# mpriessner/MultiModalSpectralTransformer

Hardware: NVIDIA B200
Metric: generated SMILES tokens/sec (higher is better)
Workload: dtype bf16

## Files before the change

multimodalspectraltransformer_b200/csrc/engine.cu:

```cuda
#include "engine.cuh"
#include "kernels_simt.cuh"
#include "kernels_tc.cuh"
#include "kernels_decode.cuh"
#include "kernels_ffn.cuh"
#include "kernels_attn5.cuh"
#include "kernels_compact.cuh"
#include "kernels_beam.cuh"
#include "kernels_smiles.cuh"
#include "kernels_retire.cuh"

#include <algorithm>
#include <cstdlib>
#include <cstring>

namespace mmt {
thread_local std::string g_last_error;

static const char* kEmbedKeys[5] = {
    "linear_spec_embedding_1H.point_embedding_layer_1H.fc_H",
    "linear_spec_embedding_13C.point_embedding_layer_13C.fc_C",
    "linear_spec_embedding_HSQC.point_embedding_layer_HSQC.fc_HSQC",
    "linear_spec_embedding_COSY.point_embedding_layer_COSY.fc_COSY",
    "linear_spec_embedding_IR.linear_spec_embedding_IR"};
static const char* kEncNames[6] = {"encoder_1H", "encoder_13C", "encoder_HSQC", "encoder_COSY", "encoder_IR", "encoder_cross"};
// ... 811 lines not shown
        }
    }
    {
        EncGroupRun g;
        memset(&g, 0, sizeof(g));
        g.X = b.Xc; g.rows = Bc * L.S_total; g.S = L.S_total; g.kbias = key_bias; g.kidx = b.kidx_c; g.nk = b.nk_c;
        g.qkv = b.QKV; g.att = b.ATT; g.part = b.PART; g.h = b.H;
        g.x16 = b.Xc16; g.att16 = b.ATT16; g.h16 = b.H16;
        for (int l = 0; l < d.n_enc_layers; ++l) {
            g.w = &e->enc[5][l];
            if (l == d.n_enc_layers - 1) { g.out = d_memory; g.out16 = nullptr; g.stride_b = 1; g.stride_s = B_total; g.off = b0; }
            if (bf16) MMT_TRY(encoder_layer_bf16(e, &g, 1, Bc, d.n_heads_cross, d.d_ff, s));
            else MMT_TRY(encoder_layer_fp32(e, &g, 1, Bc, d.n_heads_cross, d.d_ff, s));
        }
    }
    return 0;
}

struct DecBuffers {
    float *x, *qkv, *att, *part, *qc, *h;
    int64_t part_rows;
    char* kv_pool; int* block_table;
    int64_t pool_pages;
    char* cross_kv;
    size_t kv_esz;
    int *nk, *row_start; int64_t* row_off; float* kbias_c;
    int* ctl;
    uint64_t* rng_state;
    __nv_bfloat16 *x16, *att16, *h16, *mem16;
    int64_t plan_rows;
    const int *orig, *col_start, *col_count;
    int* eos_len;
    int *rt_orig[2], *rt_bt, *rt_src, *rt_col_start, *rt_col_count;
};
constexpr int MAX_SPLITS = 32;

static void plan_decoder(Arena& a, const mmt_model_desc& d, int64_t Nw, int Bmw, int S, int max_len, DecBuffers& b, bool bf16, int fused_rows, int kv_copies = 1,
                         bool retire = false) {
    const int L = d.n_dec_layers;
    const int pps = (max_len + PAGE_TOKENS - 1) / PAGE_TOKENS;
    b.x = a.get<float>(Nw * D);
    b.qkv = a.get<float>(Nw * 3 * D);
    b.att = a.get<float>(Nw * D);
    b.part_rows = std::max<int64_t>(Nw, std::min<int64_t>(Nw, std::max(fused_rows, 2048)) * MAX_SPLITS);
    b.part = a.get<float>(b.part_rows * D);
    b.qc = a.get<float>(Nw * D);
    b.h = a.get<float>(bf16 ? 0 : Nw * d.d_ff);
    b.kv_esz = bf16 ? 2 : 4;
    b.pool_pages = (int64_t)kv_copies * Nw * pps;
    b.kv_pool = a.get<char>((size_t)L * b.pool_pages * 2 * PAGE_TOKENS * D * b.kv_esz);
    b.block_table = a.get<int>(Nw * pps);
    int64_t R = (int64_t)Bmw * S;
    b.cross_kv = a.get<char>((size_t)L * 2 * R * D * b.kv_esz);
    b.nk = a.get<int>(Bmw);
    b.row_start = a.get<int>(Bmw);
    b.row_off = a.get<int64_t>(R);
    b.kbias_c = a.get<float>(R);
    b.ctl = a.get<int>(8 + 256);
    b.rng_state = a.get<uint64_t>(2);
    b.x16 = b.att16 = b.h16 = b.mem16 = nullptr;
    if (bf16) {
        b.x16 = a.get<__nv_bfloat16>(Nw * D);
        b.att16 = a.get<__nv_bfloat16>(Nw * D);
        b.h16 = nullptr;
        b.mem16 = a.get<__nv_bfloat16>(R * D);
    }
    b.plan_rows = 0; b.orig = b.col_start = b.col_count = nullptr; b.eos_len = nullptr;
    b.rt_orig[0] = b.rt_orig[1] = b.rt_bt = b.rt_src = b.rt_col_start = b.rt_col_count = nullptr;
    if (retire) {
        b.rt_orig[0] = a.get<int>(Nw); b.rt_orig[1] = a.get<int>(Nw); b.rt_bt = a.get<int>(Nw * pps); b.rt_src = a.get<int>(Nw);
        b.rt_col_start = a.get<int>(Bmw); b.rt_col_count = a.get<int>(Bmw);
    }
}

__global__ void init_block_table(int* bt, int64_t Nw, int pps) {
    int64_t i = (int64_t)blockIdx.x * blockDim.x + threadIdx.x;
    if (i < Nw * pps) bt[i] = (int)((i % pps) * Nw + i / pps);
}

struct DecodeRun {
    const mmt_decode_args* a;
    int mode;
    const int64_t* trg;
    const int64_t* target = nullptr; float* target_prob = nullptr;
    int T;
    int64_t* tokens; float* probs; float* logits;
    int64_t ldn = -1;
    bool serial_first = false;
    bool per_memory_rng = false;
    int64_t eos = -1;
    int32_t* len = nullptr;
    int64_t* h_rows = nullptr;
};

static int decode_prepare_wave(mmt_engine* e, const mmt_decode_args& a, int b0, int Bmw, DecBuffers& b, bool bf16, cudaStream_t s) {
// ... 12 lines not shown
        pack_rows_bf16<<<(unsigned)((R + 7) / 8), 256, 0, s>>>(a.d_memory + (int64_t)b0 * a.stride_b, b.row_off, 0, R, b.mem16);
        MMT_TRY(check_launch(e, "pack_rows_bf16", s));
        for (int l = 0; l < d.n_dec_layers; ++l) {
            TcGemmParams p = tc_params((int)R, 2 * D, D);
            p.bias = e->dec[l].ca_in_b + D;
            p.out_b16 = reinterpret_cast<__nv_bfloat16*>(b.cross_kv + (size_t)l * 2 * R * D * b.kv_esz);
            p.head_major = 1; p.hm_heads = d.n_heads; p.hm_dh = dh; p.hm_rows = a.S;
            MMT_TRY(launch_tc(e, p, b.mem16, D, e->Wb(e->dec[l].ca_in_w + (int64_t)D * D), TC_EPI_STORE, s, e->Wlo(e->dec[l].ca_in_w + (int64_t)D * D)));
        }
        return 0;
    }
    for (int l = 0; l < d.n_dec_layers; ++l) {
        GemmParams p = gemm_params(2 * D, D, 0, 0);
        p.g[0].A = a.d_memory + (int64_t)b0 * a.stride_b; p.g[0].a_row_off = b.row_off; p.g[0].lda = 0;
        p.g[0].W = e->dec[l].ca_in_w + (int64_t)D * D;
        p.g[0].bias = e->dec[l].ca_in_b + D;
        p.g[0].C = reinterpret_cast<float*>(b.cross_kv + (size_t)l * 2 * R * D * b.kv_esz); p.g[0].M = (int)R;
        p.out_mode = GEMM_OUT_HEADMAJOR; p.hm_heads = d.n_heads; p.hm_dh = dh; p.hm_rows = a.S;
        MMT_TRY(launch_gemm(e, p, 1, (int)R, s));
    }
    return 0;
}

static int decode_self_attention_layer(mmt_engine* e, const LayerW& w, const DecBuffers& b, char* pool, int pps, int64_t Nw, bool bf16,
                                       bool pdl_u, cudaStream_t s) {
    const int H = e->desc.n_heads, dh = D / H;
    const float scale = 1.0f / sqrtf((float)dh);
    const int* step = b.ctl;
    const int M = (int)Nw;
    if (dh != 8) MMT_FAIL("decoder head dim must be 8");
    if (bf16) {
        TcGemmParams p = tc_params(M, 3 * D, D);
        p.bias = w.in_b; p.out_f32 = b.qkv; p.ld_f32 = e->use_kv_epilogue ? D : 3 * D;
        p.kv_append = e->use_kv_epilogue ? (e->kv_tok_major && H % 8 == 0 ? 2 : 1) : 0; p.kv_pool = reinterpret_cast<__nv_bfloat16*>(pool); p.block_table = b.block_table; p.pps = pps; p.step = step; p.kv_heads = H;
        MMT_TRY(launch_tc(e, p, b.x16, D, e->Wb(w.in_w), TC_EPI_STORE, s, e->dec_proj_single ? nullptr : e->Wlo(w.in_w), pdl_u));
    } else {
        GemmParams p = gemm_params(3 * D, D, 3 * D, 0);
        p.g[0].A = b.x; p.g[0].lda = D; p.g[0].W = w.in_w; p.g[0].bias = w.in_b; p.g[0].C = b.qkv; p.g[0].M = M;
        p.splits = 1; p.part_stride = Nw * D;
        MMT_TRY(launch_gemm(e, p, 1, M, s, b.plan_rows));
    }
    prof_pre(e, s);
    const unsigned sa_blocks = (unsigned)((Nw * (H / 4) + 7) / 8);
    if (bf16 && e->use_kv_epilogue && e->kv_tok_major && H % 8 == 0)
        launch_args(decode_self_attention_tm<8>, dim3((unsigned)((Nw * (H / 8) + 7) / 8)), dim3(256), 0, s, pdl_u, (const float*)b.qkv, (const __nv_bfloat16*)reinterpret_cast<__nv_bfloat16*>(pool), (const int*)b.block_table, pps, Nw, H, scale, step, b.att16);
    else if (bf16 && e->use_kv_epilogue) launch_args(decode_self_attention_g8<8, __nv_bfloat16, false>, dim3(sa_blocks), dim3(256), 0, s, pdl_u, (const float*)b.qkv, reinterpret_cast<__nv_bfloat16*>(pool), (const int*)b.block_table, pps, Nw, H, scale, step, (float*)nullptr, b.att16);
    else if (bf16) launch_args(decode_self_attention_g8<8, __nv_bfloat16>, dim3(sa_blocks), dim3(256), 0, s, pdl_u, (const float*)b.qkv, reinterpret_cast<__nv_bfloat16*>(pool), (const int*)b.block_table, pps, Nw, H, scale, step, (float*)nullptr, b.att16);
    else decode_self_attention_g8<8, float><<<sa_blocks, 256, 0, s>>>(b.qkv, reinterpret_cast<float*>(pool), b.block_table, pps, Nw, H, scale, step, b.att, b.att16);
    return check_launch(e, "decode_self_attention", s);
}

static int decode_cross_attention_layer(mmt_engine* e, const mmt_decode_args& a, const DecBuffers& b, const char* ckv, int64_t Nw, int Bmw,
                                        bool bf16, bool pdl_u, cudaStream_t s) {
    const int H = e->desc.n_heads, dh = D / H;
    const float scale = 1.0f / sqrtf((float)dh);
    if (dh != 8) MMT_FAIL("decoder head dim must be 8");
    const unsigned attn_blocks = (unsigned)((Nw * H + 7) / 8);
    prof_pre(e, s);
    if (bf16 && a.n_cand >= 8 && e->use_tc_attention)
        launch_args(decode_cross_attention_tc, dim3(H, Bmw), dim3(256), dx_smem_bytes(a.S), s, pdl_u, (const float*)b.qc, reinterpret_cast<const __nv_bfloat16*>(ckv), (int64_t)a.S, (const int*)b.nk, (const int*)b.row_start, (const float*)b.kbias_c, (int)a.n_cand, H, scale, (float*)nullptr, b.att16, b.col_start, b.col_count);
    else if (bf16) launch_args(decode_cross_attention<8, __nv_bfloat16>, dim3(attn_blocks), dim3(256), 0, s, pdl_u, (const float*)b.qc, reinterpret_cast<const __nv_bfloat16*>(ckv), (int64_t)a.S, (const int*)b.nk, (const int*)b.row_start, (const float*)b.kbias_c, (int)a.n_cand, Nw, H, scale, (float*)nullptr, b.att16, b.orig);
    else decode_cross_attention<8, float><<<attn_blocks, 256, 0, s>>>(b.qc, reinterpret_cast<const float*>(ckv), a.S, b.nk, b.row_start, b.kbias_c, a.n_cand, Nw, H, scale, b.att, b.att16, b.orig);
    return check_launch(e, "decode_cross_attention", s);
}

struct DecOps {
    mmt_engine* e; const DecBuffers& b; int64_t Nw; bool pdl_u; cudaStream_t s;
    int64_t plan() const { return b.plan_rows > 0 ? b.plan_rows : Nw; }
// ... 129 lines not shown
        if (bf16 && e->ffn_splits_override > 0) ffn_splits = e->ffn_splits_override;
        if (!cl_ffn && (int64_t)ffn_splits * Nw > b.part_rows) MMT_FAIL("decode: FFN partial buffer too small for this wave (plan_decoder)");
        if (cl_ffn) ffn_splits = 0;
        for (int l = 0; l < d.n_dec_layers; ++l) {
            const LayerW& w = e->dec[l];
            DecAttnParams q;
            memset(&q, 0, sizeof(q));
            if (l == 0) {
                if (r.trg) { q.tokens = r.trg + n0; q.tok_shift = 0; }
                else { q.tokens = r.tokens + n0; q.tok_shift = 1; }
                q.sos = 3; q.ldn = ldn; q.E_tok = e->W("embed_trg.weight"); q.E_pos = e->W("pe_trg.weight"); q.vocab = d.vocab;
            } else {
                const LayerW& pw = e->dec[l - 1];
                q.x_in = b.x;
                if (!cl_ffn) { q.part = b.part; q.splits = ffn_splits; q.part_stride = Nw * D; q.pbias = pw.l2_b; q.pgamma = pw.n3_w; q.pbeta = pw.n3_b; }
            }
            if (cl_ffn) {
                MMT_TRY(tc_init(e));
                MMT_TRY(make_tmap(&q.tmW1, e->Wb(w.l1_w), d.d_ff, D, D));
                MMT_TRY(make_tmap(&q.tmW2, e->Wb(w.l2_w), D, d.d_ff, d.d_ff));
                q.b1 = w.l1_b; q.b2 = w.l2_b; q.n3_w = w.n3_w; q.n3_b = w.n3_b; q.x_out = b.x;
            }
            q.in_w = w.in_w; q.in_b = w.in_b; q.out_w = w.out_w; q.out_b = w.out_b; q.n1_w = w.n1_w; q.n1_b = w.n1_b;
            q.kv_pool = b.kv_pool + (size_t)l * b.pool_pages * 2 * PAGE_TOKENS * D * b.kv_esz; q.block_table = b.block_table; q.pps = pps;
            q.step = step;
            q.in_w16 = e->Wb(w.in_w); q.out_w16 = e->Wb(w.out_w); q.cq_w16 = e->Wb(w.ca_in_w); q.co_w16 = e->Wb(w.ca_out_w);
            q.cq_w = w.ca_in_w; q.cq_b = w.ca_in_b; q.co_w = w.ca_out_w; q.co_b = w.ca_out_b; q.n2_w = w.n2_w; q.n2_b = w.n2_b;
            q.ckv = b.cross_kv + (size_t)l * 2 * R * D * b.kv_esz; q.rows_total = a.S;
            q.nk = b.nk; q.row_start = b.row_start; q.kbias_c = b.kbias_c; q.n_cand = a.n_cand;
            q.x2 = b.x; q.x2_16 = bf16 ? b.x16 : nullptr; q.M = Nw; q.scale = scale; q.eps = 1e-5f;
            q.dbg = (e->da_dbg && l == 3) ? e->da_dbg : nullptr;
            prof_pre(e, s);
            const bool pdl_l = pdl && !(l == 0 && r.serial_first);
            if (cl_ffn) launch_kernel_cluster(decode_attn<8, __nv_bfloat16, true>, dim3(blocks), dim3(DA_THREADS), DA_SMEM_BYTES_CL, s, pdl_l, DA_CL, q);
            else if (bf16) launch_kernel(decode_attn<8, __nv_bfloat16>, dim3(blocks), dim3(DA_THREADS), DA_SMEM_BYTES, s, pdl_l, q);
            else launch_kernel(decode_attn<8, float>, dim3(blocks), dim3(DA_THREADS), DA_SMEM_BYTES, s, pdl_l, q);
            MMT_TRY(check_launch(e, "decode_attn", s));
            if (cl_ffn) continue;
            if (bf16) {
                FfnParams f = ffn_params(M, d.d_ff);
                f.b1 = w.l1_b; f.splits = ffn_splits; f.out_f32 = b.part; f.part_stride = Nw * D;
                f.dbg = (e->da_dbg && l == 3) ? e->da_dbg + 2048 * 16 : nullptr;
                MMT_TRY(launch_ffn(e, f, b.x16, D, e->Wb(w.l1_w), o.dlo(w.l1_w), e->Wb(w.l2_w), o.dlo(w.l2_w), TC_EPI_STORE, s, pdl));
            } else {
                MMT_TRY(o.gemm(b.x, D, w.l1_w, w.l1_b, b.h, d.d_ff, D, 1, 1));
                MMT_TRY(o.gemm(b.h, d.d_ff, w.l2_w, nullptr, b.part, D, d.d_ff, 0, ffn_splits));
            }
        }
    } else {
        prof_pre(e, s);
        if (r.trg) launch_args(decode_embed, dim3((unsigned)((Nw + 3) / 4)), dim3(128), 0, s, pdl_u, r.trg + n0, 0, 3, Nw, ldn, e->W("embed_trg.weight"), e->W("pe_trg.weight"), (int)d.vocab, step, b.x, b.x16, b.orig);
        else launch_args(decode_embed, dim3((unsigned)((Nw + 3) / 4)), dim3(128), 0, s, pdl_u, (const int64_t*)(r.tokens + n0), 1, 3, Nw, ldn, e->W("embed_trg.weight"), e->W("pe_trg.weight"), (int)d.vocab, step, b.x, b.x16, b.orig);
        MMT_TRY(check_launch(e, "decode_embed", s));

        for (int l = 0; l < d.n_dec_layers; ++l) {
            const LayerW& w = e->dec[l];
            char* pool = b.kv_pool + (size_t)l * b.pool_pages * 2 * PAGE_TOKENS * D * b.kv_esz;
            const char* ckv = b.cross_kv + (size_t)l * 2 * R * D * b.kv_esz;
            MMT_TRY(decode_self_attention_layer(e, w, b, pool, pps, Nw, bf16, pdl_u, s));
            MMT_TRY(decode_self_tail_layer(o, w, bf16));
            MMT_TRY(decode_cross_attention_layer(e, a, b, ckv, Nw, Bmw, bf16, pdl_u, s));
            MMT_TRY(decode_cross_tail_layer(o, w, l, bf16));
        }
    }
    SampleParams sp;
    memset(&sp, 0, sizeof(sp));
    sp.x = b.x; sp.W = e->W("fc_out.weight"); sp.b = e->W("fc_out.bias"); sp.V = d.vocab; sp.N = Nw; sp.ldn = ldn;
    sp.temperature = a.temperature; sp.mode = r.mode;
    int smc = a.rng_sm_count > 0 ? a.rng_sm_count : e->sm_count;
    int mts = a.rng_max_threads_per_sm > 0 ? a.rng_max_threads_per_sm : e->max_threads_per_sm;
    int64_t Nrng = r.per_memory_rng ? a.n_cand : (a.N_total > 0 ? a.N_total : N_total);
    sp.rng.seed = a.philox_seed; sp.rng.offset = a.philox_offset; sp.rng.numel = Nrng * d.vocab;
    sp.rng.threads = torch_rng_threads(sp.rng.numel, smc, mts);
    sp.rng_inc = torch_rng_increment(sp.rng.numel, smc, mts);
    sp.rng_dev = b.rng_state;
    sp.seq_index_base = a.seq_index_base + n0;
    if (r.per_memory_rng) { sp.rng_cand = a.n_cand; sp.rng_col_steps = a.max_len; }
    sp.tokens = r.tokens ? r.tokens + n0 : nullptr; sp.probs = r.probs ? r.probs + n0 : nullptr;
    sp.logits = r.logits ? r.logits + n0 * d.vocab : nullptr;
    sp.target = r.target ? r.target + n0 : nullptr; sp.target_prob = r.target_prob ? r.target_prob + n0 : nullptr;
    sp.ctl.step = b.ctl; sp.ctl.done_ctas = b.ctl + 1; sp.ctl.nonpad = (r.mode == 0) ? b.ctl + 8 : nullptr;
    sp.advance = 1;
// ... 26 lines not shown
    const int64_t N_total = (int64_t)a.Bm * a.n_cand;
    const int64_t max_wave_seqs = e->max_wave_seqs > 0 ? e->max_wave_seqs
                                  : (a.precision == MMT_PREC_BF16 ? (int64_t)e->sm_count * (e->total_mem >= ((size_t)128 << 30) ? 8 : 4) * 128 : 32768);
    int Bm_wave = (int)std::max<int64_t>(1, std::min<int64_t>(a.Bm, max_wave_seqs / a.n_cand));
    const int n_waves = (a.Bm + Bm_wave - 1) / Bm_wave;
    if (a.precision != MMT_PREC_FP32 && a.precision != MMT_PREC_BF16) MMT_FAIL("decode: bad precision");
    const bool bf16 = a.precision == MMT_PREC_BF16;
    constexpr int MAX_LANES = 4;
    int NL = 1;
    {
        const int64_t Nwave = (int64_t)Bm_wave * a.n_cand;
        const bool fused = e->fused_decode_rows > 0 && Nwave <= e->fused_decode_rows;
        if (fused && e->use_graph && !e->profiling) {
            NL = std::min(std::min(e->decode_lanes, MAX_LANES), Bm_wave);
            while (NL > 1 && Nwave / NL < 32) --NL;
        } else if (!fused && bf16 && e->use_graph && !e->profiling && Nwave >= 4096) {
            NL = std::min(std::min(e->decode_lanes_large, MAX_LANES), Bm_wave);
        }
    }
    const int Bm_lane = (Bm_wave + NL - 1) / NL;
    const bool retire = r.eos >= 0;
    const bool small_wave = e->fused_decode_rows > 0 && (int64_t)Bm_wave * a.n_cand <= e->fused_decode_rows;
    const bool staged = e->use_graph && e->use_graph_cache && !e->profiling && n_waves == 1 && r.mode != 2 && !r.trg && (!retire || small_wave);
    Arena ar;
    DecBuffers lb[MAX_LANES];
    int64_t* st_tokens = nullptr; float* st_probs = nullptr;
    int* eos_all = nullptr;
    auto plan_all = [&]() {
        for (int i = 0; i < NL; ++i) plan_decoder(ar, d, (int64_t)Bm_lane * a.n_cand, Bm_lane, a.S, a.max_len, lb[i], bf16, e->fused_decode_rows, 1, retire);
        if (staged) { st_tokens = ar.get<int64_t>((size_t)a.max_len * N_total); st_probs = ar.get<float>((size_t)a.max_len * N_total); }
        if (retire) eos_all = ar.get<int>(N_total);
    };
    ar.plan = true;
    plan_all();
    MMT_TRY(ensure_arena(e, ar.off));
    ar.plan = false; ar.base = e->arena; ar.cap = e->arena_bytes; ar.off = 0;
    plan_all();
    DecodeRun rs = r;
    if (staged) { rs.tokens = st_tokens; rs.probs = r.probs ? st_probs : nullptr; }
    const int pps = (a.max_len + PAGE_TOKENS - 1) / PAGE_TOKENS;
    const bool early = (r.mode == 0) && a.stop_on_all_pad && n_waves == 1;
    int steps_done = r.T;
    std::vector<int64_t> nonpad_total(r.T, 0);
    std::vector<int64_t> live_total(r.T, 0), rows_at(r.T, 0);
    if (retire) {
        fill_i32<<<(unsigned)((N_total + 255) / 256), 256, 0, s>>>(eos_all, N_total, a.max_len);
        MMT_CUDA(cudaGetLastError());
        for (int i = 0; i < 2; ++i) if (!e->poll_ev[i]) MMT_CUDA(cudaEventCreateWithFlags(&e->poll_ev[i], cudaEventDisableTiming));
    }
    for (int wv = 0; wv < n_waves; ++wv) {
        const int wb0 = wv * Bm_wave;
        const int Bmw = std::min(Bm_wave, a.Bm - wb0);
// ... 379 lines not shown
    if (prop.major != 10) MMT_FAIL(std::string("device is sm_") + std::to_string(prop.major * 10 + prop.minor) + "; this library is built for sm_100a (B200) only");
    MMT_CUDA(cudaSetDevice(device));
    mmt_engine* e = new mmt_engine();
    e->desc = *desc; e->device = device; e->sm_count = prop.multiProcessorCount; e->max_threads_per_sm = prop.maxThreadsPerMultiProcessor; e->total_mem = prop.totalGlobalMem;
    e->reg = build_registry(*desc);
    if (getenv("MMT_NO_GRAPH")) e->use_graph = false;
    if (getenv("MMT_NO_PDL")) e->use_pdl = false;
    if (getenv("MMT_NO_GRAPH_CACHE")) e->use_graph_cache = false;
    if (const char* v = getenv("MMT_GRAPH_STEPS")) e->graph_steps = std::max(1, atoi(v));
    if (getenv("MMT_NO_ENC_STREAMS")) e->use_enc_streams = false;
    if (const char* v = getenv("MMT_DECODE_LANES")) e->decode_lanes = std::max(1, atoi(v));
    if (getenv("MMT_DENSE_ENCODER")) e->use_compact = false;
    if (getenv("MMT_NO_TC_ATTENTION")) e->use_tc_attention = false;
    if (getenv("MMT_TC5_ATTENTION")) e->use_tc5_attention = true;
    if (const char* v = getenv("MMT_FFN_SPLITS")) { int k = atoi(v); if (k == 1 || k == 2 || k == 4 || k == 8 || k == 16 || k == 32) e->ffn_splits_override = k; }
    if (getenv("MMT_TC_ATTENTION_FP32")) e->tc_attention_fp32 = true;
    if (const char* v = getenv("MMT_FUSED_DECODE_ROWS")) e->fused_decode_rows = atoi(v);
    if (getenv("MMT_DEC_FFN_TWO_TERM")) e->dec_ffn_single = false;
    if (getenv("MMT_DEC_PROJ_TWO_TERM")) e->dec_proj_single = false;
    if (const char* v = getenv("MMT_PDL_ROWS")) e->pdl_rows = atoi(v);
    if (getenv("MMT_NO_GEMM_CHAIN")) e->use_gemm_chain = false;
    if (getenv("MMT_NO_FFN_WIDE")) e->use_ffn_wide = false;
    if (getenv("MMT_NO_KV_EPILOGUE")) e->use_kv_epilogue = false;
    if (getenv("MMT_KV_HEAD_MAJOR")) e->kv_tok_major = false;
    if (getenv("MMT_CLUSTER_FFN")) e->use_cluster_ffn = true;
    if (getenv("MMT_NO_FFN_PROLOGUE")) e->use_ffn_prologue = false;
    if (getenv("MMT_ENC_FFN_SINGLE")) e->enc_ffn_single = true;
    if (const char* v = getenv("MMT_DECODE_LANES_LARGE")) e->decode_lanes_large = std::max(1, atoi(v));
    if (const char* v = getenv("MMT_MAX_WAVE_SEQS")) e->max_wave_seqs = std::max(1, atoi(v));
    if (n_floats != e->reg.total) { delete e; MMT_FAIL("weight blob has " + std::to_string(n_floats) + " floats, expected " + std::to_string(build_registry(*desc).total)); }
    auto fail = [&](const std::string& m) { mmt_destroy(e); g_last_error = m; return 1; };
    if (cudaMalloc(&e->w32, n_floats * sizeof(float)) != cudaSuccess) return fail("cudaMalloc weights failed");
    if (cudaMalloc(&e->w16, n_floats * sizeof(__nv_bfloat16)) != cudaSuccess) return fail("cudaMalloc bf16 weights failed");
    if (cudaMemcpy(e->w32, h_weights, n_floats * sizeof(float), cudaMemcpyHostToDevice) != cudaSuccess) return fail("weight H2D copy failed");
    if (cudaMalloc(&e->w16lo, n_floats * sizeof(__nv_bfloat16)) != cudaSuccess) return fail("cudaMalloc bf16 weights (low term) failed");
    f32_to_bf16_split<<<(unsigned)((n_floats + 255) / 256), 256>>>(e->w32, n_floats, e->w16, e->w16lo);
    if (cudaDeviceSynchronize() != cudaSuccess) return fail(std::string("bf16 weight conversion failed: ") + cudaGetErrorString(cudaGetLastError()));
    if (cudaMallocHost(&e->h_pinned, 2048 * sizeof(int32_t)) != cudaSuccess) return fail("cudaMallocHost failed");
    for (int k = 0; k < 6; ++k) {
        e->enc[k].resize(desc->n_enc_layers);
        for (int l = 0; l < desc->n_enc_layers; ++l) fill_layer(e, e->enc[k][l], std::string(kEncNames[k]) + ".layers." + std::to_string(l), false);
    }
    e->dec.resize(desc->n_dec_layers);
    for (int l = 0; l < desc->n_dec_layers; ++l) fill_layer(e, e->dec[l], "decoder.layers." + std::to_string(l), true);
    *out = e;
    return 0;
}

void mmt_destroy(mmt_engine* e) {
    if (!e) return;
    cudaSetDevice(e->device);
    cudaDeviceSynchronize();
    if (e->w32) cudaFree(e->w32);
    if (e->w16) cudaFree(e->w16);
    if (e->w16lo) cudaFree(e->w16lo);
    if (e->arena) cudaFree(e->arena);
    if (e->h_pinned) cudaFreeHost(e->h_pinned);
    for (auto& c : e->graph_cache) cudaGraphExecDestroy(c.exec);
    for (int i = 0; i < 5; ++i) if (e->enc_stream[i]) cudaStreamDestroy(e->enc_stream[i]);
    for (int i = 0; i < 6; ++i) if (e->enc_ev[i]) cudaEventDestroy(e->enc_ev[i]);
    for (int i = 0; i < 4; ++i) { if (e->cap_stream[i]) cudaStreamDestroy(e->cap_stream[i]); if (e->lane_ev[i]) cudaEventDestroy(e->lane_ev[i]); }
    for (int i = 0; i < 2; ++i) if (e->poll_ev[i]) cudaEventDestroy(e->poll_ev[i]);
    if (e->last_use) cudaEventDestroy(e->last_use);
    delete e;
}

int32_t mmt_memory_len(const mmt_model_desc* desc, uint32_t mode_bits) {
    if (check_desc(desc)) return -1;
    return mode_layout(*desc, mode_bits).S_total;
}
int32_t mmt_mask_is_float(uint32_t mode_bits) {
    for (int m = 0; m < 4; ++m) if (!((mode_bits >> m) & 1)) return 1;
    return 0;
}

int32_t mmt_encode(mmt_engine* e, const mmt_spectra* in, int32_t B, uint32_t mode_bits, int32_t precision,
                   float* d_memory, float* d_embedding_src, float* d_key_bias, uint8_t* d_pad_mask,
                   float* d_fingerprint, float* d_avg_memory, void* stream) {
    if (!e || !in) MMT_FAIL("null engine / spectra");
// ... 652 lines not shown
```

multimodalspectraltransformer_b200/csrc/engine.cuh:

```cuda
#pragma once
#include <mutex>
#include <string>
#include <unordered_map>
#include <vector>

#include "../../include/mmt_b200.h"
#include "common.cuh"

namespace mmt {

extern thread_local std::string g_last_error;

#define MMT_FAIL(msg)                                                                   \
    do {                                                                                \
        ::mmt::g_last_error = std::string(__FILE__) + ":" + std::to_string(__LINE__) + ": " + (msg); \
        return 1;                                                                       \
    } while (0)
#define MMT_CUDA(call)                                                                  \
    do {                                                                                \
        cudaError_t err__ = (call);                                                     \
        if (err__ != cudaSuccess) MMT_FAIL(std::string(#call) + " -> " + cudaGetErrorString(err__)); \
    } while (0)
#define MMT_TRY(call)                                                                   \
    do {                                                                                \
// ... 74 lines not shown

}

struct mmt_engine {
    mmt_model_desc desc;
    int device = 0, sm_count = 0, max_threads_per_sm = 0;
    size_t total_mem = 0;
    mmt::Registry reg;
    float* w32 = nullptr;
    __nv_bfloat16* w16 = nullptr;
    __nv_bfloat16* w16lo = nullptr;
    std::vector<mmt::LayerW> enc[6];
    std::vector<mmt::LayerW> dec;
    char* arena = nullptr;
    size_t arena_bytes = 0;
    int64_t launches = 0;
    bool use_graph = true;
    int fused_decode_rows = 2048;
    int max_wave_seqs = 0;
    bool enc_ffn_single = false;
    bool use_ffn_prologue = true;
    bool use_cluster_ffn = false;
    bool kv_tok_major = true;
    bool use_kv_epilogue = true;
    bool use_ffn_wide = true;
    bool use_gemm_chain = true;
    bool dec_proj_single = true;
    bool sample_ready = false;
    bool dec_ffn_single = true;
    bool use_compact = true;
    struct GraphEntry { std::vector<uint64_t> key; cudaGraphExec_t exec; int64_t launches_per_group; uint64_t stamp; };
    std::vector<GraphEntry> graph_cache;
    uint64_t graph_cache_clock = 0;
    bool use_graph_cache = true;
    bool use_tc_attention = true;
    bool use_tc5_attention = false;
    bool tc_attention_fp32 = false;
    int ffn_splits_override = 0;
    bool use_enc_streams = true;
    cudaStream_t enc_stream[5] = {nullptr, nullptr, nullptr, nullptr, nullptr};
    cudaEvent_t enc_ev[6] = {nullptr, nullptr, nullptr, nullptr, nullptr, nullptr};
    int graph_steps = 16;
    int pdl_rows = 4096;
    bool use_pdl = true;
    cudaStream_t cap_stream[4] = {nullptr, nullptr, nullptr, nullptr};
    cudaEvent_t lane_ev[4] = {nullptr, nullptr, nullptr, nullptr};
// ... 23 lines not shown
```

multimodalspectraltransformer_b200/csrc/kernels_simt.cuh:

```cuda
#pragma once
#include "common.cuh"
#include "philox.cuh"

namespace mmt {

constexpr int GEMM_MAX_GROUPS = 6;

struct GemmGroup {
    const float* A;
    const int64_t* a_row_off;
    const float* W;
    const float* bias;
    float* C;
    const int* M_dev;
    int64_t lda;
    int M;
};

enum { GEMM_OUT_ROWMAJOR = 0, GEMM_OUT_HEADMAJOR = 1 };

struct GemmParams {
    GemmGroup g[GEMM_MAX_GROUPS];
    int N, K;
    int splits;
// ... 760 lines not shown
        unsigned m = __ballot_sync(0xffffffffu, valid);
        if (valid) {
            int pos = b * p.S + count + __popc(m & ((1u << lane) - 1));
            p.row_off[pos] = (int64_t)j * p.stride_s + (int64_t)b * p.stride_b;
            p.kbias_c[pos] = bias;
        }
        count += __popc(m);
    }
    for (int jj = count + lane; jj < p.S; jj += 32) {
        p.row_off[b * p.S + jj] = (int64_t)b * p.stride_b;
        p.kbias_c[b * p.S + jj] = MMT_NEG_INF;
    }
    if (lane == 0) { p.nk[b] = count; p.row_start[b] = b * p.S; }
}

struct StepCtl {
    int* step;
    int* done_ctas;
    int* nonpad;
};

__global__ void __launch_bounds__(128) decode_embed(const int64_t* tokens, int tok_shift, int sos, int64_t N, int64_t ldn,
                                                    const float* E_tok, const float* E_pos, int vocab,
                                                    const int* step, float* x, __nv_bfloat16* x_bf16, const int* orig) {
    pdl_launch_dependents();
    pdl_wait();
    const int t = *step;
    const int64_t n = (int64_t)blockIdx.x * 4 + (threadIdx.x >> 5);
    if (n >= N) return;
    const int lane = threadIdx.x & 31;
    const int64_t col = orig ? orig[n] : n;
    int64_t tok;
    if (tok_shift) tok = (t == 0) ? sos : tokens[(int64_t)(t - 1) * ldn + col];
    else tok = tokens[(int64_t)t * ldn + col];
    if (tok < 0 || tok >= vocab) tok = 0;
    float4 a = *reinterpret_cast<const float4*>(E_tok + tok * D + lane * 4);
    float4 b = *reinterpret_cast<const float4*>(E_pos + (int64_t)t * D + lane * 4);
    float4 o = make_float4(a.x + b.x, a.y + b.y, a.z + b.z, a.w + b.w);
    *reinterpret_cast<float4*>(x + n * D + lane * 4) = o;
    if (x_bf16) {
        __nv_bfloat162 lo = __floats2bfloat162_rn(o.x, o.y), hi = __floats2bfloat162_rn(o.z, o.w);
        *reinterpret_cast<uint2*>(x_bf16 + n * D + lane * 4) =
            make_uint2(*reinterpret_cast<uint32_t*>(&lo), *reinterpret_cast<uint32_t*>(&hi));
    }
}

template <int DH, typename KVT>
__global__ void __launch_bounds__(256) decode_self_attention(const float* qkv, KVT* kv_pool, const int* block_table,
                                                             int pages_per_seq, int64_t N, int H, float scale,
                                                             const int* step, float* out, __nv_bfloat16* out16) {
    static_assert(DH == 8, "8-element key rows");
    typedef KvRow<KVT> KV;
    const int t = *step;
    const int64_t w = (int64_t)blockIdx.x * 8 + (threadIdx.x >> 5);
    if (w >= N * H) return;
    const int lane = threadIdx.x & 31;
    const int64_t n = w / H;
    const int h = (int)(w % H);
// ... 125 lines not shown
    }
    float Mx = m;
    Mx = fmaxf(Mx, __shfl_xor_sync(0xffffffffu, Mx, 1)); Mx = fmaxf(Mx, __shfl_xor_sync(0xffffffffu, Mx, 2)); Mx = fmaxf(Mx, __shfl_xor_sync(0xffffffffu, Mx, 4));
    const float corr = (m == MMT_NEG_INF) ? 0.f : expf(m - Mx);
    l *= corr;
    l += __shfl_xor_sync(0xffffffffu, l, 1); l += __shfl_xor_sync(0xffffffffu, l, 2); l += __shfl_xor_sync(0xffffffffu, l, 4);
#pragma unroll
    for (int d = 0; d < DH; ++d) acc[d] *= corr;
#pragma unroll
    for (int off = 4; off >= 1; off >>= 1) {
        const bool up = (lane & off) != 0;
#pragma unroll
        for (int i = 0; i < off; ++i) {
            const float send = up ? acc[i] : acc[i + off];
            const float keep = up ? acc[i + off] : acc[i];
            acc[i] = keep + __shfl_xor_sync(0xffffffffu, send, off);
        }
    }
    const float o = acc[0] / l;
    if (out) out[n * D + h * DH + kl] = o;
    if (out16) out16[n * D + h * DH + kl] = __float2bfloat16_rn(o);
}

template <int DH>
__global__ void __launch_bounds__(256) decode_self_attention_tm(const float* qd, const __nv_bfloat16* kv_pool, const int* block_table,
                                                                int pages_per_seq, int64_t N, int H, float scale,
                                                                const int* step, __nv_bfloat16* out16) {
    static_assert(DH == 8, "8-element key rows");
    typedef KvRow<__nv_bfloat16> KV;
    pdl_launch_dependents();
    pdl_wait();
    const int t = *step;
    const int HG = H / 8;
    const int64_t w = (int64_t)blockIdx.x * 8 + (threadIdx.x >> 5);
    if (w >= N * HG) return;
    const int lane = threadIdx.x & 31, h8 = lane >> 2, kl = lane & 3;
    const int64_t n = w / HG;
    const int h = (int)(w % HG) * 8 + h8;
    constexpr int PAGE_ELEMS = 2 * PAGE_TOKENS * D;
    const int* bt = block_table + n * pages_per_seq;
    const float* row = qd + n * D + h * DH;
    float q[DH], acc[DH];
    {
        const float4 a = *reinterpret_cast<const float4*>(row), b = *reinterpret_cast<const float4*>(row + 4);
        q[0] = a.x * scale; q[1] = a.y * scale; q[2] = a.z * scale; q[3] = a.w * scale;
        q[4] = b.x * scale; q[5] = b.y * scale; q[6] = b.z * scale; q[7] = b.w * scale;
    }
#pragma unroll
    for (int d = 0; d < DH; ++d) acc[d] = 0.f;
    float m = MMT_NEG_INF, l = 0.f;
    auto row_ptr = [&](int j) { return kv_pool + (int64_t)bt[j / PAGE_TOKENS] * PAGE_ELEMS + (j % PAGE_TOKENS) * (2 * D) + h * DH; };
    typename KV::Raw rk0, rk1, rv0, rv1;
    if (kl <= t) {
        const __nv_bfloat16* p0 = row_ptr(kl);
        const __nv_bfloat16* p1 = row_ptr(kl + 4 <= t ? kl + 4 : kl);
        rk0 = KV::ld(p0); rk1 = KV::ld(p1);
        rv0 = KV::ld(p0 + D); rv1 = KV::ld(p1 + D);
    }
    for (int j0 = kl; j0 <= t; j0 += 8) {
        const bool has1 = j0 + 4 <= t;
        const typename KV::Raw ck0 = rk0, ck1 = rk1, cv0 = rv0, cv1 = rv1;
        const int jn = j0 + 8;
        if (jn <= t) {
            const __nv_bfloat16* p0 = row_ptr(jn);
            const __nv_bfloat16* p1 = row_ptr(jn + 4 <= t ? jn + 4 : jn);
            rk0 = KV::ld(p0); rk1 = KV::ld(p1);
            rv0 = KV::ld(p0 + D); rv1 = KV::ld(p1 + D);
        }
        float k0[DH], k1[DH];
        KV::unpack(ck0, k0); KV::unpack(ck1, k1);
        float s0 = 0.f, s1 = 0.f;
#pragma unroll
        for (int d = 0; d < DH; ++d) { s0 = fmaf(q[d], k0[d], s0); s1 = fmaf(q[d], k1[d], s1); }
        if (!has1) s1 = MMT_NEG_INF;
// ... 11 lines not shown
        KV::unpack(cv0, v0); KV::unpack(cv1, v1);
#pragma unroll
        for (int d = 0; d < DH; ++d) acc[d] = fmaf(e1, v1[d], fmaf(e0, v0[d], acc[d]));
    }
    float Mx = m;
    Mx = fmaxf(Mx, __shfl_xor_sync(0xffffffffu, Mx, 1)); Mx = fmaxf(Mx, __shfl_xor_sync(0xffffffffu, Mx, 2));
    const float corr = (m == MMT_NEG_INF) ? 0.f : expf(m - Mx);
    l *= corr;
    l += __shfl_xor_sync(0xffffffffu, l, 1); l += __shfl_xor_sync(0xffffffffu, l, 2);
#pragma unroll
    for (int d = 0; d < DH; ++d) acc[d] *= corr;
#pragma unroll
    for (int off = 2; off >= 1; off >>= 1) {
        const bool up = (lane & off) != 0;
#pragma unroll
        for (int i = 0; i < 2 * off; ++i) {
            const float send = up ? acc[i] : acc[i + 2 * off];
            const float keep = up ? acc[i + 2 * off] : acc[i];
            acc[i] = keep + __shfl_xor_sync(0xffffffffu, send, off);
        }
    }
    const __nv_bfloat162 o = __floats2bfloat162_rn(acc[0] / l, acc[1] / l);
    *reinterpret_cast<__nv_bfloat162*>(out16 + n * D + h * DH + 2 * kl) = o;
}

template <int DH, typename KVT>
__global__ void __launch_bounds__(256) decode_cross_attention(const float* q_in, const KVT* kv, int64_t rows_total,
                                                              const int* nk, const int* row_start, const float* kbias_c,
                                                              int n_cand, int64_t N, int H, float scale, float* out,
                                                              __nv_bfloat16* out16, const int* orig) {
    static_assert(DH == 8, "8-element key rows");
    typedef KvRow<KVT> KV;
    pdl_launch_dependents();
    pdl_wait();
    const int64_t w = (int64_t)blockIdx.x * 8 + (threadIdx.x >> 5);
    if (w >= N * H) return;
    const int lane = threadIdx.x & 31;
    const int64_t n = w / H;
    const int h = (int)(w % H);
    const int64_t b = (orig ? orig[n] : n) / n_cand;
    const int cnt = nk[b];
    const int64_t r0 = row_start[b];
    const int64_t S = rows_total;
    const KVT* Kh = kv + (((int64_t)b * 2 + 0) * H + h) * S * DH;
    const KVT* Vh = kv + (((int64_t)b * 2 + 1) * H + h) * S * DH;
    const float* bias = kbias_c + r0;
// ... 495 lines not shown
```

Measured before the change: 17.41 million.

## Precompute layer-0 decoder self-attention QKV table indexed by position and token

Layer-0 decoder input is just token embedding plus positional embedding, so its Q/K/V projection depends only on (position, token). A table of Q (fp32) and K/V (bf16) for every (t, token) pair is built once per engine and reused. The decode embed kernel records a per-sequence token history, and the layer-0 attention reads Q and K/V rows from the table through that history. This removes the per-step layer-0 QKV GEMM and its KV-cache pool writes and memory, at the cost of a one-time table build that cannot run under graph capture, plus extra gather indirection in attention.

```diff
diff --git a/multimodalspectraltransformer_b200/csrc/engine.cu b/multimodalspectraltransformer_b200/csrc/engine.cu
--- a/multimodalspectraltransformer_b200/csrc/engine.cu
+++ b/multimodalspectraltransformer_b200/csrc/engine.cu
@@ -857,6 +857,8 @@
     int64_t part_rows;
     char* kv_pool; int* block_table;
     int64_t pool_pages;
+    int kv_first;
+    uint8_t* hist; int hist_ld;
     char* cross_kv;
     size_t kv_esz;
     int *nk, *row_start; int64_t* row_off; float* kbias_c;
@@ -871,7 +873,7 @@
 constexpr int MAX_SPLITS = 32;
 
 static void plan_decoder(Arena& a, const mmt_model_desc& d, int64_t Nw, int Bmw, int S, int max_len, DecBuffers& b, bool bf16, int fused_rows, int kv_copies = 1,
-                         bool retire = false) {
+                         bool retire = false, bool l0_table = false, bool l0_pool = true) {
     const int L = d.n_dec_layers;
     const int pps = (max_len + PAGE_TOKENS - 1) / PAGE_TOKENS;
     b.x = a.get<float>(Nw * D);
@@ -883,7 +885,10 @@
     b.h = a.get<float>(bf16 ? 0 : Nw * d.d_ff);
     b.kv_esz = bf16 ? 2 : 4;
     b.pool_pages = (int64_t)kv_copies * Nw * pps;
-    b.kv_pool = a.get<char>((size_t)L * b.pool_pages * 2 * PAGE_TOKENS * D * b.kv_esz);
+    b.kv_first = l0_pool ? 0 : 1;
+    b.kv_pool = a.get<char>((size_t)(L - b.kv_first) * b.pool_pages * 2 * PAGE_TOKENS * D * b.kv_esz);
+    b.hist_ld = pps * PAGE_TOKENS;
+    b.hist = l0_table ? a.get<uint8_t>((size_t)Nw * b.hist_ld) : nullptr;
     b.block_table = a.get<int>(Nw * pps);
     int64_t R = (int64_t)Bmw * S;
     b.cross_kv = a.get<char>((size_t)L * 2 * R * D * b.kv_esz);
@@ -906,6 +911,10 @@
         b.rt_orig[0] = a.get<int>(Nw); b.rt_orig[1] = a.get<int>(Nw); b.rt_bt = a.get<int>(Nw * pps); b.rt_src = a.get<int>(Nw);
         b.rt_col_start = a.get<int>(Bmw); b.rt_col_count = a.get<int>(Bmw);
     }
+}
+
+static char* layer_pool(const DecBuffers& b, int l) {
+    return l < b.kv_first ? nullptr : b.kv_pool + (size_t)(l - b.kv_first) * b.pool_pages * 2 * PAGE_TOKENS * D * b.kv_esz;
 }
 
 __global__ void init_block_table(int* bt, int64_t Nw, int pps) {
@@ -964,13 +973,65 @@
     return 0;
 }
 
+static int ensure_l0_table(mmt_engine* e, cudaStream_t s) {
+    if (e->l0_qtab) return 0;
+    cudaStreamCaptureStatus cs;
+    MMT_CUDA(cudaStreamIsCapturing(s, &cs));
+    if (cs != cudaStreamCaptureStatusNone) MMT_FAIL("decode: the layer-0 table is built by the first large bf16 decode, which cannot run under stream capture");
+    const mmt_model_desc& d = e->desc;
+    const LayerW& w = e->dec[0];
+    const int64_t rows = (int64_t)d.max_len * d.vocab;
+    __nv_bfloat16* x16 = nullptr;
+    float* qkv = nullptr;
+    float* qtab = nullptr;
+    __nv_bfloat16* kvtab = nullptr;
+    auto release = [&]() { cudaFree(x16); cudaFree(qkv); cudaFree(qtab); cudaFree(kvtab); };
+    if (cudaMalloc(&x16, rows * D * sizeof(__nv_bfloat16)) != cudaSuccess || cudaMalloc(&qkv, rows * 3 * D * sizeof(float)) != cudaSuccess ||
+        cudaMalloc(&qtab, rows * D * sizeof(float)) != cudaSuccess || cudaMalloc(&kvtab, rows * 2 * D * sizeof(__nv_bfloat16)) != cudaSuccess) {
+        release();
+        MMT_FAIL("decode: cudaMalloc of the layer-0 table failed");
+    }
+    int rc = 0;
+    prof_pre(e, s);
+    l0_table_rows<<<(unsigned)((rows + 3) / 4), 128, 0, s>>>(e->W("embed_trg.weight"), e->W("pe_trg.weight"), (int)d.vocab, rows, x16);
+    rc = check_launch(e, "l0_table_rows", s);
+    if (!rc) {
+        TcGemmParams p = tc_params((int)rows, 3 * D, D);
+        p.bias = w.in_b; p.out_f32 = qkv; p.ld_f32 = 3 * D;
+        rc = launch_tc(e, p, x16, D, e->Wb(w.in_w), TC_EPI_STORE, s, e->dec_proj_single ? nullptr : e->Wlo(w.in_w));
+    }
+    if (!rc) {
+        prof_pre(e, s);
+        l0_table_split<<<(unsigned)((rows + 3) / 4), 128, 0, s>>>(qkv, rows, qtab, kvtab);
+        rc = check_launch(e, "l0_table_split", s);
+    }
+    cudaError_t se = cudaStreamSynchronize(s);
+    cudaFree(x16); cudaFree(qkv);
+    x16 = nullptr; qkv = nullptr;
+    if (rc || se != cudaSuccess) {
+        release();
+        if (rc) return rc;
+        MMT_FAIL(std::string("decode: layer-0 table build failed: ") + cudaGetErrorString(se));
+    }
+    e->l0_qtab = qtab; e->l0_kvtab = kvtab;
+    return 0;
+}
+
 static int decode_self_attention_layer(mmt_engine* e, const LayerW& w, const DecBuffers& b, char* pool, int pps, int64_t Nw, bool bf16,
-                                       bool pdl_u, cudaStream_t s) {
+                                       bool pdl_u, cudaStream_t s, bool l0_table = false) {
     const int H = e->desc.n_heads, dh = D / H;
     const float scale = 1.0f / sqrtf((float)dh);
     const int* step = b.ctl;
     const int M = (int)Nw;
     if (dh != 8) MMT_FAIL("decoder head dim must be 8");
+    const unsigned tm_blocks = (unsigned)((Nw * (H / 8) + 7) / 8);
+    if (l0_table) {
+        if (!b.hist || !e->l0_qtab) MMT_FAIL("decode: layer-0 table path without its table or token history");
+        const TmTable src{e->l0_qtab, e->l0_kvtab, b.hist, b.hist_ld, (int)e->desc.vocab, b.orig};
+        prof_pre(e, s);
+        launch_args(decode_self_attention_tm<8, TmTable>, dim3(tm_blocks), dim3(256), 0, s, pdl_u, src, Nw, H, scale, step, b.att16);
+        return check_launch(e, "decode_self_attention_l0", s);
+    }
     if (bf16) {
         TcGemmParams p = tc_params(M, 3 * D, D);
         p.bias = w.in_b; p.out_f32 = b.qkv; p.ld_f32 = e->use_kv_epilogue ? D : 3 * D;
@@ -985,7 +1046,7 @@
     prof_pre(e, s);
     const unsigned sa_blocks = (unsigned)((Nw * (H / 4) + 7) / 8);
     if (bf16 && e->use_kv_epilogue && e->kv_tok_major && H % 8 == 0)
-        launch_args(decode_self_attention_tm<8>, dim3((unsigned)((Nw * (H / 8) + 7) / 8)), dim3(256), 0, s, pdl_u, (const float*)b.qkv, (const __nv_bfloat16*)reinterpret_cast<__nv_bfloat16*>(pool), (const int*)b.block_table, pps, Nw, H, scale, step, b.att16);
+        launch_args(decode_self_attention_tm<8, TmPaged>, dim3(tm_blocks), dim3(256), 0, s, pdl_u, TmPaged{b.qkv, reinterpret_cast<const __nv_bfloat16*>(pool), b.block_table, pps}, Nw, H, scale, step, b.att16);
     else if (bf16 && e->use_kv_epilogue) launch_args(decode_self_attention_g8<8, __nv_bfloat16, false>, dim3(sa_blocks), dim3(256), 0, s, pdl_u, (const float*)b.qkv, reinterpret_cast<__nv_bfloat16*>(pool), (const int*)b.block_table, pps, Nw, H, scale, step, (float*)nullptr, b.att16);
     else if (bf16) launch_args(decode_self_attention_g8<8, __nv_bfloat16>, dim3(sa_blocks), dim3(256), 0, s, pdl_u, (const float*)b.qkv, reinterpret_cast<__nv_bfloat16*>(pool), (const int*)b.block_table, pps, Nw, H, scale, step, (float*)nullptr, b.att16);
     else decode_self_attention_g8<8, float><<<sa_blocks, 256, 0, s>>>(b.qkv, reinterpret_cast<float*>(pool), b.block_table, pps, Nw, H, scale, step, b.att, b.att16);
@@ -1161,7 +1222,8 @@
                 q.b1 = w.l1_b; q.b2 = w.l2_b; q.n3_w = w.n3_w; q.n3_b = w.n3_b; q.x_out = b.x;
             }
             q.in_w = w.in_w; q.in_b = w.in_b; q.out_w = w.out_w; q.out_b = w.out_b; q.n1_w = w.n1_w; q.n1_b = w.n1_b;
-            q.kv_pool = b.kv_pool + (size_t)l * b.pool_pages * 2 * PAGE_TOKENS * D * b.kv_esz; q.block_table = b.block_table; q.pps = pps;
+            q.kv_pool = layer_pool(b, l); q.block_table = b.block_table; q.pps = pps;
+            if (!q.kv_pool) MMT_FAIL("decode: fused step without layer-0 cache pages (run_decode planned every wave on the layer-0 table)");
             q.step = step;
             q.in_w16 = e->Wb(w.in_w); q.out_w16 = e->Wb(w.out_w); q.cq_w16 = e->Wb(w.ca_in_w); q.co_w16 = e->Wb(w.ca_out_w);
             q.cq_w = w.ca_in_w; q.cq_b = w.ca_in_b; q.co_w = w.ca_out_w; q.co_b = w.ca_out_b; q.n2_w = w.n2_w; q.n2_b = w.n2_b;
@@ -1187,16 +1249,17 @@
             }
         }
     } else {
+        const bool l0_table = b.hist != nullptr;
+        __nv_bfloat16* x16 = l0_table ? nullptr : b.x16;
         prof_pre(e, s);
-        if (r.trg) launch_args(decode_embed, dim3((unsigned)((Nw + 3) / 4)), dim3(128), 0, s, pdl_u, r.trg + n0, 0, 3, Nw, ldn, e->W("embed_trg.weight"), e->W("pe_trg.weight"), (int)d.vocab, step, b.x, b.x16, b.orig);
-        else launch_args(decode_embed, dim3((unsigned)((Nw + 3) / 4)), dim3(128), 0, s, pdl_u, (const int64_t*)(r.tokens + n0), 1, 3, Nw, ldn, e->W("embed_trg.weight"), e->W("pe_trg.weight"), (int)d.vocab, step, b.x, b.x16, b.orig);
+        if (r.trg) launch_args(decode_embed, dim3((unsigned)((Nw + 3) / 4)), dim3(128), 0, s, pdl_u, r.trg + n0, 0, 3, Nw, ldn, e->W("embed_trg.weight"), e->W("pe_trg.weight"), (int)d.vocab, step, b.x, x16, b.orig, b.hist, b.hist_ld);
+        else launch_args(decode_embed, dim3((unsigned)((Nw + 3) / 4)), dim3(128), 0, s, pdl_u, (const int64_t*)(r.tokens + n0), 1, 3, Nw, ldn, e->W("embed_trg.weight"), e->W("pe_trg.weight"), (int)d.vocab, step, b.x, x16, b.orig, b.hist, b.hist_ld);
         MMT_TRY(check_launch(e, "decode_embed", s));
 
         for (int l = 0; l < d.n_dec_layers; ++l) {
             const LayerW& w = e->dec[l];
-            char* pool = b.kv_pool + (size_t)l * b.pool_pages * 2 * PAGE_TOKENS * D * b.kv_esz;
             const char* ckv = b.cross_kv + (size_t)l * 2 * R * D * b.kv_esz;
-            MMT_TRY(decode_self_attention_layer(e, w, b, pool, pps, Nw, bf16, pdl_u, s));
+            MMT_TRY(decode_self_attention_layer(e, w, b, layer_pool(b, l), pps, Nw, bf16, pdl_u, s, l == 0 && l0_table));
             MMT_TRY(decode_self_tail_layer(o, w, bf16));
             MMT_TRY(decode_cross_attention_layer(e, a, b, ckv, Nw, Bmw, bf16, pdl_u, s));
             MMT_TRY(decode_cross_tail_layer(o, w, l, bf16));
@@ -1269,12 +1332,25 @@
     const bool retire = r.eos >= 0;
     const bool small_wave = e->fused_decode_rows > 0 && (int64_t)Bm_wave * a.n_cand <= e->fused_decode_rows;
     const bool staged = e->use_graph && e->use_graph_cache && !e->profiling && n_waves == 1 && r.mode != 2 && !r.trg && (!retire || small_wave);
+    bool l0_table = false, l0_pool = true;
+    if (bf16 && e->use_l0_table && e->use_kv_epilogue && e->kv_tok_major && d.n_heads % 8 == 0 && d.vocab <= 256) {
+        bool any_fused = false;
+        for (int wb0 = 0; wb0 < a.Bm; wb0 += Bm_wave)
+            for (int i = 0; i < NL; ++i) {
+                const int Bmw = std::min(Bm_wave, a.Bm - wb0), lo = std::min(i * Bm_lane, Bmw), hi = std::min(lo + Bm_lane, Bmw);
+                if (hi <= lo) continue;
+                if (e->fused_decode_rows > 0 && (int64_t)(hi - lo) * a.n_cand <= e->fused_decode_rows) any_fused = true;
+                else l0_table = true;
+            }
+        l0_pool = any_fused;
+    }
+    if (l0_table) MMT_TRY(ensure_l0_table(e, s));
     Arena ar;
     DecBuffers lb[MAX_LANES];
     int64_t* st_tokens = nullptr; float* st_probs = nullptr;
     int* eos_all = nullptr;
     auto plan_all = [&]() {
-        for (int i = 0; i < NL; ++i) plan_decoder(ar, d, (int64_t)Bm_lane * a.n_cand, Bm_lane, a.S, a.max_len, lb[i], bf16, e->fused_decode_rows, 1, retire);
+        for (int i = 0; i < NL; ++i) plan_decoder(ar, d, (int64_t)Bm_lane * a.n_cand, Bm_lane, a.S, a.max_len, lb[i], bf16, e->fused_decode_rows, 1, retire, l0_table, l0_pool);
         if (staged) { st_tokens = ar.get<int64_t>((size_t)a.max_len * N_total); st_probs = ar.get<float>((size_t)a.max_len * N_total); }
         if (retire) eos_all = ar.get<int>(N_total);
     };
@@ -1700,6 +1776,7 @@
     if (getenv("MMT_NO_GEMM_CHAIN")) e->use_gemm_chain = false;
     if (getenv("MMT_NO_FFN_WIDE")) e->use_ffn_wide = false;
     if (getenv("MMT_NO_KV_EPILOGUE")) e->use_kv_epilogue = false;
+    if (getenv("MMT_NO_L0_TABLE")) e->use_l0_table = false;
     if (getenv("MMT_KV_HEAD_MAJOR")) e->kv_tok_major = false;
     if (getenv("MMT_CLUSTER_FFN")) e->use_cluster_ffn = true;
     if (getenv("MMT_NO_FFN_PROLOGUE")) e->use_ffn_prologue = false;
@@ -1733,6 +1810,8 @@
     if (e->w16) cudaFree(e->w16);
     if (e->w16lo) cudaFree(e->w16lo);
     if (e->arena) cudaFree(e->arena);
+    if (e->l0_qtab) cudaFree(e->l0_qtab);
+    if (e->l0_kvtab) cudaFree(e->l0_kvtab);
     if (e->h_pinned) cudaFreeHost(e->h_pinned);
     for (auto& c : e->graph_cache) cudaGraphExecDestroy(c.exec);
     for (int i = 0; i < 5; ++i) if (e->enc_stream[i]) cudaStreamDestroy(e->enc_stream[i]);
diff --git a/multimodalspectraltransformer_b200/csrc/engine.cuh b/multimodalspectraltransformer_b200/csrc/engine.cuh
--- a/multimodalspectraltransformer_b200/csrc/engine.cuh
+++ b/multimodalspectraltransformer_b200/csrc/engine.cuh
@@ -120,6 +120,9 @@
     bool use_ffn_prologue = true;
     bool use_cluster_ffn = false;
     bool kv_tok_major = true;
+    bool use_l0_table = true;
+    float* l0_qtab = nullptr;
+    __nv_bfloat16* l0_kvtab = nullptr;
     bool use_kv_epilogue = true;
     bool use_ffn_wide = true;
     bool use_gemm_chain = true;
diff --git a/multimodalspectraltransformer_b200/csrc/kernels_simt.cuh b/multimodalspectraltransformer_b200/csrc/kernels_simt.cuh
--- a/multimodalspectraltransformer_b200/csrc/kernels_simt.cuh
+++ b/multimodalspectraltransformer_b200/csrc/kernels_simt.cuh
@@ -806,7 +806,8 @@
 
 __global__ void __launch_bounds__(128) decode_embed(const int64_t* tokens, int tok_shift, int sos, int64_t N, int64_t ldn,
                                                     const float* E_tok, const float* E_pos, int vocab,
-                                                    const int* step, float* x, __nv_bfloat16* x_bf16, const int* orig) {
+                                                    const int* step, float* x, __nv_bfloat16* x_bf16, const int* orig,
+                                                    uint8_t* hist, int hist_ld) {
     pdl_launch_dependents();
     pdl_wait();
     const int t = *step;
@@ -818,6 +819,7 @@
     if (tok_shift) tok = (t == 0) ? sos : tokens[(int64_t)(t - 1) * ldn + col];
     else tok = tokens[(int64_t)t * ldn + col];
     if (tok < 0 || tok >= vocab) tok = 0;
+    if (hist && lane == 0) hist[col * hist_ld + t] = (uint8_t)tok;
     float4 a = *reinterpret_cast<const float4*>(E_tok + tok * D + lane * 4);
     float4 b = *reinterpret_cast<const float4*>(E_pos + (int64_t)t * D + lane * 4);
     float4 o = make_float4(a.x + b.x, a.y + b.y, a.z + b.z, a.w + b.w);
@@ -989,9 +991,30 @@
     if (out16) out16[n * D + h * DH + kl] = __float2bfloat16_rn(o);
 }
 
-template <int DH>
-__global__ void __launch_bounds__(256) decode_self_attention_tm(const float* qd, const __nv_bfloat16* kv_pool, const int* block_table,
-                                                                int pages_per_seq, int64_t N, int H, float scale,
+struct TmPaged {
+    const float* qd; const __nv_bfloat16* kv_pool; const int* block_table; int pps;
+    struct Seq {
+        const float* q; const __nv_bfloat16* pool; const int* bt;
+        __device__ __forceinline__ const float* q_row(int) const { return q; }
+        __device__ __forceinline__ const __nv_bfloat16* kv_row(int j) const {
+            return pool + (int64_t)bt[j / PAGE_TOKENS] * (2 * PAGE_TOKENS * D) + (j % PAGE_TOKENS) * (2 * D);
+        }
+    };
+    __device__ __forceinline__ Seq seq(int64_t n) const { return {qd + n * D, kv_pool, block_table + n * pps}; }
+};
+struct TmTable {
+    const float* qtab; const __nv_bfloat16* kvtab; const uint8_t* hist; int hist_ld; int vocab; const int* orig;
+    struct Seq {
+        const float* qtab; const __nv_bfloat16* kvtab; const uint8_t* hist; int vocab;
+        __device__ __forceinline__ const float* q_row(int t) const { return qtab + ((int64_t)t * vocab + hist[t]) * D; }
+        __device__ __forceinline__ const __nv_bfloat16* kv_row(int j) const { return kvtab + ((int64_t)j * vocab + hist[j]) * (2 * D); }
+    };
+    __device__ __forceinline__ Seq seq(int64_t n) const {
+        return {qtab, kvtab, hist + (int64_t)(orig ? orig[n] : n) * hist_ld, vocab};
+    }
+};
+template <int DH, class Src>
+__global__ void __launch_bounds__(256) decode_self_attention_tm(const Src src, int64_t N, int H, float scale,
                                                                 const int* step, __nv_bfloat16* out16) {
     static_assert(DH == 8, "8-element key rows");
     typedef KvRow<__nv_bfloat16> KV;
@@ -1004,9 +1027,8 @@
     const int lane = threadIdx.x & 31, h8 = lane >> 2, kl = lane & 3;
     const int64_t n = w / HG;
     const int h = (int)(w % HG) * 8 + h8;
-    constexpr int PAGE_ELEMS = 2 * PAGE_TOKENS * D;
-    const int* bt = block_table + n * pages_per_seq;
-    const float* row = qd + n * D + h * DH;
+    const typename Src::Seq sq = src.seq(n);
+    const float* row = sq.q_row(t) + h * DH;
     float q[DH], acc[DH];
     {
         const float4 a = *reinterpret_cast<const float4*>(row), b = *reinterpret_cast<const float4*>(row + 4);
@@ -1016,7 +1038,7 @@
 #pragma unroll
     for (int d = 0; d < DH; ++d) acc[d] = 0.f;
     float m = MMT_NEG_INF, l = 0.f;
-    auto row_ptr = [&](int j) { return kv_pool + (int64_t)bt[j / PAGE_TOKENS] * PAGE_ELEMS + (j % PAGE_TOKENS) * (2 * D) + h * DH; };
+    auto row_ptr = [&](int j) { return sq.kv_row(j) + h * DH; };
     typename KV::Raw rk0, rk1, rv0, rv1;
     if (kl <= t) {
         const __nv_bfloat16* p0 = row_ptr(kl);
@@ -1074,6 +1096,32 @@
     }
     const __nv_bfloat162 o = __floats2bfloat162_rn(acc[0] / l, acc[1] / l);
     *reinterpret_cast<__nv_bfloat162*>(out16 + n * D + h * DH + 2 * kl) = o;
+}
+
+__global__ void __launch_bounds__(128) l0_table_rows(const float* E_tok, const float* E_pos, int vocab, int64_t rows, __nv_bfloat16* out) {
+    const int64_t r = (int64_t)blockIdx.x * 4 + (threadIdx.x >> 5);
+    if (r >= rows) return;
+    const int lane = threadIdx.x & 31;
+    const int64_t t = r / vocab, tok = r % vocab;
+    const float4 a = *reinterpret_cast<const float4*>(E_tok + tok * D + lane * 4);
+    const float4 b = *reinterpret_cast<const float4*>(E_pos + t * D + lane * 4);
+    const float4 o = make_float4(a.x + b.x, a.y + b.y, a.z + b.z, a.w + b.w);
+    __nv_bfloat162 lo = __floats2bfloat162_rn(o.x, o.y), hi = __floats2bfloat162_rn(o.z, o.w);
+    *reinterpret_cast<uint2*>(out + r * D + lane * 4) = make_uint2(*reinterpret_cast<uint32_t*>(&lo), *reinterpret_cast<uint32_t*>(&hi));
+}
+
+__global__ void __launch_bounds__(128) l0_table_split(const float* qkv, int64_t rows, float* qtab, __nv_bfloat16* kvtab) {
+    const int64_t r = (int64_t)blockIdx.x * 4 + (threadIdx.x >> 5);
+    if (r >= rows) return;
+    const int lane = threadIdx.x & 31;
+    const float* src = qkv + r * (3 * D);
+    *reinterpret_cast<float4*>(qtab + r * D + lane * 4) = *reinterpret_cast<const float4*>(src + lane * 4);
+#pragma unroll
+    for (int c = 0; c < 2; ++c) {
+        const float4 v = *reinterpret_cast<const float4*>(src + D + c * D + lane * 4);
+        __nv_bfloat162 lo = __floats2bfloat162_rn(v.x, v.y), hi = __floats2bfloat162_rn(v.z, v.w);
+        *reinterpret_cast<uint2*>(kvtab + r * (2 * D) + c * D + lane * 4) = make_uint2(*reinterpret_cast<uint32_t*>(&lo), *reinterpret_cast<uint32_t*>(&hi));
+    }
 }
 
 template <int DH, typename KVT>
```

Result: faster. 18.11 million (median of 6 runs) (+4.0%).
